# esteinig/sketchy

Measured on AMD Instinct MI355X. Metric: reads/sec streamed (s=10000,k=16,40k-genome ref), higher is better.
Workload: dtype u64

## Files before the change

sketchy_amd/csrc/skx_capi.hip:

```cpp
#include <dlfcn.h>
#include <hip/hip_runtime.h>
#include <rccl/rccl.h>

#include <unistd.h>

#include <algorithm>
#include <atomic>
#include <chrono>
#include <cmath>
#include <condition_variable>
#include <cstdarg>
#include <cstdio>
#include <cstdlib>
#include <cstring>
#include <mutex>
#include <string>
#include <thread>
#include <unordered_map>
#include <vector>

#include "sketchy_hip.h"
#include "skx_common.hpp"
#include "skx_genome_groups.hpp"
#include "skx_kernels.hpp"
// ... 985 lines not shown
    u32 *d_hist = nullptr, *d_nprow = nullptr;
    u64* d_pcw = nullptr;
    u32 npat_pad = 0;
    skx::PatRows pat_rows() const { return skx::PatRows{d_hist, npat_pad, d_gain_l, d_nprow}; }
    skx::RareIndex rare_index() const {
        skx::RareIndex ri = ref->rare_index();
        if (!use_pat) { ri.prec = nullptr; ri.n_pat = 0; }
        if (!static_dense) { ri.qs = nullptr; ri.n_sd = 0; }
        return ri;
    }
    u32 *d_cbad = nullptr, *d_nqc = nullptr;
    u32 *d_spc_g0 = nullptr, *d_spc_grp = nullptr;
    u32 n_pad_c = 0, n_grp_c = 0, cand_seq = 0;
    struct PassSet {
        u64 *tab = nullptr;
        u32 *cand = nullptr;
        u64 *tabc = nullptr;
        u32 *ncand = nullptr;
        u32 *mode = nullptr, *any_full = nullptr, *nqc_total = nullptr;
        u32 *ext = nullptr;
        skx::SlotExtents smap_ext;
        u32 mqc_whole = 0xFFu;
        u64 *mc = nullptr;
        u64 *mqc = nullptr;
        u64 *rowany_c = nullptr;
        u32 *grp_any_c = nullptr;
        u32 *smap = nullptr;
        u32 *pair_qc = nullptr;
        u32 *nd = nullptr;
        u32 *h_pub = nullptr;
    } ps[2];
    struct PassChains {
        bool pending = false, ranked = false, has_cand = false, update_table = false, forced_full = false, legacy = false;
        SubPass subs[kGroupMax];
        int n_sub = 0, b = 0, slot = 0;
        u32 P = 0, nq_rows = 0, seq = 0;
        u64 nq_est = 0;
    } pcq[2];
    int pc_head = 0, pc_n = 0;
    bool hint_all_overflow = false;
    u32 hint_seq = 0;
    u32 passes_since_fresh = 0;
    bool fresh_table = true;
    u32 legacy_run = 0;
    u64 batches_compact = 0, batches_full = 0;
    bool have_split_hint = false;
    double nd_frac = 1.0;
    u32 qcap_max = 0;
    bool qcap_auto = false;
    u64 qrows_grown = 0;
    u32 coalesce = 1;
    u32 rpass = 0;
    u64 reads_total = 0;
    uint8_t* d_bases = nullptr;
    u64* d_offsets = nullptr;
    u64* d_sk = nullptr;
    u32 *d_len = nullptr, *d_cnt = nullptr, *d_poff = nullptr;
    bool side_ready[kSides] = {};
    u64* sd_sk[kSides] = {};
    u64 pool_cap[kSides] = {};
    u32 pool_fixed = 0;
    u64* sd_rows[kSides] = {};
    u32 cur_stride = 0;
    u32 cur_pool_cap = 0, cur_pool_fixed = 0;
    u32 *sd_len[kSides] = {}, *sd_cnt[kSides] = {}, *sd_poff[kSides] = {}, *sd_big[kSides] = {};
    u32 *sd_chk[kSides] = {}, *sd_retry[kSides] = {};
// ... 9 lines not shown
    bool m_filled[2] = {false, false};
    u32* d_mdirty_s = nullptr;
    u32 sd64 = 0;
    u32 qhash_cap() const { return qcap - sd64; }
    struct RankLane {
        hipStream_t s = nullptr;
        u32 *d_inc = nullptr;
        u32 *d_csum_raw = nullptr;
        u32 *d_csum = nullptr;
        u32 *d_rel = nullptr;
        u32 *d_leader = nullptr;
        u64 *d_lead_val = nullptr;
        u64 *d_gmax = nullptr;
        u64 *d_lpart_sum = nullptr;
        u32 *d_lpart_idx = nullptr;
        u32 *d_live_ctr = nullptr;
        u64 *d_lead_seg = nullptr;
        unsigned char *d_has = nullptr;
        unsigned char *d_live = nullptr;
        u64 *d_cand_sum = nullptr;
        u32 *d_cand_idx = nullptr;
        u64 *d_cum_sink = nullptr;
        u32 *d_chg_flag = nullptr, *d_chg_pos = nullptr, *d_chg_bsum = nullptr, *d_chg_codes = nullptr;
        u32 *d_call_flag = nullptr, *d_call_pos = nullptr, *d_call_bsum = nullptr, *d_call_key = nullptr;
        u32 *d_call_sp = nullptr, *d_call_idx = nullptr, *d_call_codes = nullptr;
        u64* d_call_sum = nullptr;
        u32 call_key_w = 0;
        hipEvent_t ev_cum = nullptr;
        hipEvent_t ev_done = nullptr;
        bool ready = false;
    };
    static const int kRankLanes = kRankLanesMax;
    RankLane lane[kRankLanes];
    int n_lanes = 1;
    bool own_lane_stream = false;
    u32 n_cand_units = 0;
    u64 rank_seq = 0;
    RankLane* cum_writer = nullptr;
    u64* d_tab[kRankLanes + 1] = {};
    int tab_cur = 0;
    u64* d_cum = nullptr;
    u32* d_topk_idx = nullptr;
    u64* d_topk_sum = nullptr;
    u32* bound_cons = nullptr;
    u32* d_cons = nullptr;
    ChangeOut bound_chg;
    ChangeOut d_ev;
    CallOut bound_call;
    CallOut d_call;
    u64* d_tab_tmp = nullptr;
    u32* d_rank_idx = nullptr;
    u64* d_rank_sum = nullptr;
    u32 rank_cap = 0;
    StreamStats stats;
    u32* h_poff = nullptr;
    u64* h_offsets = nullptr;
    u64* d_ht[2] = {nullptr, nullptr};
    u32 ht_slots = 0;
    u32 *d_slot_off = nullptr, *d_bcount = nullptr, *d_bbase = nullptr, *d_btot = nullptr, *d_dict_ctr[2] = {nullptr, nullptr};
    u32* d_chk = nullptr;
    u32* h_chk = nullptr;
    u32* h_chk_base = nullptr;
    u32 pub_seq = 0;
    bool chk_dirty[kSides] = {};
    u64* d_rowany[2] = {nullptr, nullptr};
    u32* d_mqext = nullptr;
// ... 18 lines not shown
        u32 n_reads = 0;
        u64 n_bases = 0, ticket = 0;
        u32* out_idx = nullptr;
        u64* out_sum = nullptr;
        u32* out_cons = nullptr;
        u32* d_cons = nullptr;
        ChangeOut out_chg;
        ChangeOut d_ev;
        u32* h_ev_n = nullptr;
        CallOut out_call;
        CallOut d_call;
        u32* h_cev_n = nullptr;
        u32* d_rows_idx = nullptr;
        u64* d_rows_sum = nullptr;
        uint8_t* d_bases = nullptr;
        u64 *d_offsets = nullptr, *h_offsets = nullptr;
        hipEvent_t ev_copy = nullptr, ev_done = nullptr;
    } slot[kSlotsMax];
    u32 n_slots = 3;
    hipStream_t hs_copy = nullptr;
    u64 next_ticket = 0;
    u32* h_nq = nullptr;
    u32 hint_pairs[2] = {0, 0};
    double nq_per_pair = 1.0;
    bool have_hint = false;
    int profiling = 0;
    std::vector<TimedSpan> spans;
    std::vector<hipEvent_t> ev_pool;
    double ms[SKX_N_STAGES] = {0, 0, 0, 0, 0};
    u64 launches[SKX_N_STAGES] = {0, 0, 0, 0, 0};
};

static void free_side(skx_stream* st, int i);
static void free_lane(skx_stream* st, int i);
static void free_call(CallOut& d) {
    void* ptrs[] = {d.sp, d.idx, d.sum, d.codes, d.n_events, d.ev_read, d.ev_sp, d.ev_idx, d.ev_sum, d.ev_codes};
    for (void* q : ptrs) (void)hipFree(q);
    d = CallOut{};
}
static void stream_free(skx_stream* st) {
    if (!st) return;
    (void)hipSetDevice(st->device);
    if (st->hs0) (void)hipStreamSynchronize(st->hs0);
    if (st->hs1) (void)hipStreamSynchronize(st->hs1);
    if (st->hs) (void)hipStreamSynchronize(st->hs);
    if (st->hs2) (void)hipStreamSynchronize(st->hs2);
    for (int i = 1; i < skx_stream::kRankLanes; ++i)
        if (st->lane[i].s) (void)hipStreamSynchronize(st->lane[i].s);
    for (int i = 0; i < kSides; ++i) (void)hipFree(st->sd_rows[i]);
    void* ptrs[] = {st->d_bases, st->d_offsets, st->d_pair_h[0], st->d_pair_h[1],
                    st->d_q[0], st->d_q[1], st->d_pair_r[0], st->d_pair_r[1], st->d_pair_q[0], st->d_pair_q[1],
                    st->d_poff_pass[0], st->d_poff_pass[1], st->d_poff_pass[2], st->d_pair_r[2], st->d_nq[0], st->d_nq[1], st->d_win[0], st->d_win[1], st->d_m, st->d_mint, st->d_mq[0], st->d_mq[1],
                    st->d_topk_idx, st->d_topk_sum, st->d_cons, st->d_ev.n_events, st->d_ev.ev_read, st->d_ev.ev_idx, st->d_ev.ev_sum, st->d_ev.ev_codes, st->d_tab_tmp, st->d_rank_idx, st->d_rank_sum, st->d_bsum, st->d_grp_any[0],
                    st->d_grp_any[1], st->d_hbuf, st->d_wb[0], st->d_wb[1], st->d_rowany[0], st->d_rowany[1], st->d_mqext,
                    st->d_qd, st->d_qrow, st->d_sslot, st->d_qinfo, st->d_qloc, st->d_cls_bsum, st->d_nd_hs,
                    st->d_rowcnt, st->d_gain, st->d_gain_s, st->d_candslot, st->d_candmask, st->d_lrow, st->d_gop, st->d_gop_pairs, st->d_nlrow, st->d_gain_l, st->d_cbase, st->d_cwl, st->d_ncwl, st->d_cw, st->d_cbad, st->d_nqc, st->d_spc_g0, st->d_spc_grp, st->d_inb, st->d_hit, st->d_hist, st->d_nprow, st->d_pcw, st->d_ms[0], st->d_ms[1], st->d_mdirty_s};
    for (auto& q : st->ps) {
        for (void* x : {(void*)q.tab, (void*)q.cand, (void*)q.tabc, (void*)q.ncand, (void*)q.mode, (void*)q.any_full, (void*)q.nqc_total, (void*)q.mc, (void*)q.mqc,
                        (void*)q.rowany_c, (void*)q.grp_any_c, (void*)q.smap, (void*)q.pair_qc, (void*)q.nd}) (void)hipFree(x);
        if (q.h_pub) (void)hipHostFree(q.h_pub);
    }
    for (auto& t : st->d_tab) (void)hipFree(t);
    for (int i = 0; i < skx_stream::kRankLanes; ++i) free_lane(st, i);
    for (int i = 1; i < skx_stream::kRankLanes; ++i)
        if (st->own_lane_stream && st->lane[i].s) (void)hipStreamDestroy(st->lane[i].s);
    for (void* p : ptrs) (void)hipFree(p);
    stats_free(st->stats);
    if (st->h_poff) (void)hipHostFree(st->h_poff);
    if (st->h_offsets) (void)hipHostFree(st->h_offsets);
    if (st->h_nq) (void)hipHostFree(st->h_nq);
    if (st->h_nd) (void)hipHostFree(st->h_nd);
    if (st->h_nq_sink) (void)hipHostFree(st->h_nq_sink);
    if (st->h_lcount) (void)hipHostFree(st->h_lcount);
    if (st->h_chk_base) (void)hipHostFree(st->h_chk_base);
    for (int i = 0; i < kSides; ++i) {
        free_side(st, i);
        if (st->ev_main[i]) (void)hipEventDestroy(st->ev_main[i]);
    }
    if (!st->shared_queues && st->hs1 && st->hs1 != st->hs0) (void)hipStreamDestroy(st->hs1);
    (void)hipFree(st->d_ht[0]); (void)hipFree(st->d_ht[1]); (void)hipFree(st->d_dict_ctr[0]); (void)hipFree(st->d_dict_ctr[1]);
    (void)hipFree(st->d_slot_off); (void)hipFree(st->d_bcount); (void)hipFree(st->d_bbase);
    (void)hipFree(st->d_btot);
    free_call(st->d_call);
    for (auto& sl : st->slot) {
        free_call(sl.d_call);
        if (sl.h_cev_n) (void)hipHostFree(sl.h_cev_n);
        (void)hipFree(sl.d_bases); (void)hipFree(sl.d_offsets); (void)hipFree(sl.d_rows_idx); (void)hipFree(sl.d_rows_sum); (void)hipFree(sl.d_cons);
        (void)hipFree(sl.d_ev.n_events); (void)hipFree(sl.d_ev.ev_read); (void)hipFree(sl.d_ev.ev_idx); (void)hipFree(sl.d_ev.ev_sum); (void)hipFree(sl.d_ev.ev_codes);
        if (sl.h_ev_n) (void)hipHostFree(sl.h_ev_n);
        if (sl.h_offsets) (void)hipHostFree(sl.h_offsets);
        if (sl.ev_copy) (void)hipEventDestroy(sl.ev_copy);
        if (sl.ev_done) (void)hipEventDestroy(sl.ev_done);
    }
    if (st->hs_copy) (void)hipStreamDestroy(st->hs_copy);
    for (auto& sp : st->spans) { (void)hipEventDestroy(sp.a); (void)hipEventDestroy(sp.b); }
    for (auto ev : st->ev_pool) (void)hipEventDestroy(ev);
// ... 60 lines not shown
        if ((e = hipMalloc(&lr.list, (size_t)lr.long_cap * 4)) != hipSuccess) return e;
        if ((e = hipMalloc(&lr.seg0, (size_t)lr.long_cap * 4)) != hipSuccess) return e;
        if ((e = hipMalloc(&lr.seg_tab, (size_t)lr.segs_cap * 4)) != hipSuccess) return e;
        if ((e = hipMalloc(&lr.seg_cnt, (size_t)lr.segs_cap * 4)) != hipSuccess) return e;
        if ((e = hipMalloc(&lr.seg_h, (size_t)lr.segs_cap * skx::long_read_seg_slots() * 8)) != hipSuccess) return e;
    }
    return hipMemset(st->sd_big[i], 0, 4);
}
static hipError_t use_side(skx_stream* st, int i) {
    if (!st->side_ready[i]) {
        hipError_t e = alloc_side(st, i);
        if (e == hipSuccess) e = hipDeviceSynchronize();
        if (e != hipSuccess) return e;
    }
    st->side = i;
    st->d_sk = st->sd_sk[i]; st->cur_stride = 0; st->cur_pool_cap = (u32)st->pool_cap[i]; st->cur_pool_fixed = st->pool_fixed;
    st->d_len = st->sd_len[i]; st->d_cnt = st->sd_cnt[i]; st->d_poff = st->sd_poff[i];
    st->d_big = st->sd_big[i]; st->d_retry = st->sd_retry[i]; st->d_chk = st->sd_chk[i];
    st->lr = st->sd_lr[i];
    st->h_chk = st->h_chk_base + 16 * i;
    return hipSuccess;
}

static hipError_t use_rows(skx_stream* st) {
    const int i = st->side;
    if (!st->sd_rows[i]) {
        hipError_t e = hipMalloc(&st->sd_rows[i], (size_t)st->max_reads * st->sk_stride * 8);
        if (e != hipSuccess) return e;
    }
    st->d_sk = st->sd_rows[i]; st->cur_stride = st->sk_stride; st->cur_pool_cap = 0; st->cur_pool_fixed = 0;
    return hipSuccess;
}

static hipError_t alloc_lane_parts(skx_stream* st, int i) {
    skx_stream::RankLane& L = st->lane[i];
    const skx_ref* ref = st->ref;
    const u32 n_sp = ref->n_species, top_k = st->top_k, n_pad = std::max<u32>(ref->n_pad, n_sp * skx::kCandCap);
    const u32 n_seg_max = (st->rpass + skx::kSegLen - 1) / skx::kSegLen, n_chunk_max = (n_seg_max + 15) / 16;
    const u32 k1 = std::max<u32>(top_k, 1);
    hipError_t e;
#define LCHK(expr) do { if ((e = (expr)) != hipSuccess) return e; } while (0)
    LCHK(hipMalloc(&L.d_inc, (size_t)n_seg_max * n_pad * 4));
    LCHK(hipMalloc(&L.d_rel, (size_t)n_seg_max * n_pad * 4));
    LCHK(hipMalloc(&L.d_live, (size_t)n_seg_max * (n_pad / 64)));
    LCHK(hipMalloc(&L.d_has, (size_t)n_seg_max * (n_pad / (skx::kRankWords * 64))));
    LCHK(hipMalloc(&L.d_lead_seg, (size_t)n_seg_max * n_sp * 8 + 64));
    LCHK(hipMalloc(&L.d_live_ctr, 8));
    LCHK(hipMemset(L.d_live_ctr, 0, 8));
    LCHK(hipMalloc(&L.d_csum, (size_t)n_chunk_max * n_pad * 4));
    LCHK(hipMalloc(&L.d_csum_raw, (size_t)n_chunk_max * n_pad * 4));
    LCHK(hipMalloc(&L.d_leader, (size_t)n_chunk_max * n_sp * k1 * 4 + 64));
    LCHK(hipMalloc(&L.d_lead_val, (size_t)n_chunk_max * n_sp * 8 + 64));
    LCHK(hipMalloc(&L.d_lpart_sum, (size_t)n_chunk_max * n_sp * skx::rank_leader_parts() * k1 * 8 + 64));
    LCHK(hipMalloc(&L.d_lpart_idx, (size_t)n_chunk_max * n_sp * skx::rank_leader_parts() * k1 * 4 + 64));
    LCHK(hipMalloc(&L.d_gmax, (size_t)(n_chunk_max + 1) * (n_pad / 256) * 8 + 64));
    if (top_k) {
        LCHK(hipMalloc(&L.d_cand_sum, (size_t)st->rpass * st->n_cand_units * top_k * 8));
        LCHK(hipMalloc(&L.d_cand_idx, (size_t)st->rpass * st->n_cand_units * top_k * 4));
    }
    LCHK(hipMalloc(&L.d_cum_sink, (size_t)n_pad * 8));
    LCHK(hipEventCreateWithFlags(&L.ev_cum, hipEventDisableTiming));
    LCHK(hipEventCreateWithFlags(&L.ev_done, hipEventDisableTiming));
#undef LCHK
    return hipSuccess;
}
static void free_lane(skx_stream* st, int i) {
    skx_stream::RankLane& L = st->lane[i];
    void* ptrs[] = {L.d_inc, L.d_rel, L.d_live, L.d_has, L.d_lead_seg, L.d_live_ctr, L.d_csum, L.d_csum_raw, L.d_leader, L.d_lead_val,
                    L.d_lpart_sum, L.d_lpart_idx, L.d_gmax, L.d_cand_sum, L.d_cand_idx, L.d_cum_sink,
                    L.d_chg_flag, L.d_chg_pos, L.d_chg_bsum, L.d_chg_codes,
                    L.d_call_flag, L.d_call_pos, L.d_call_bsum, L.d_call_key, L.d_call_sp, L.d_call_idx, L.d_call_codes, L.d_call_sum};
    for (void* q : ptrs) (void)hipFree(q);
    if (L.ev_cum) (void)hipEventDestroy(L.ev_cum);
    if (L.ev_done) (void)hipEventDestroy(L.ev_done);
    const hipStream_t keep = L.s;
    L = skx_stream::RankLane{};
    L.s = keep;
}
static hipError_t alloc_lane(skx_stream* st, int i) {
    const hipError_t e = alloc_lane_parts(st, i);
    if (e != hipSuccess) { free_lane(st, i); (void)hipGetLastError(); }
    else st->lane[i].ready = true;
    return e;
}

static int stream_create_internal(skx_stream** out, const skx_ref* ref, u32 top_k, u32 max_reads, u64 max_bases,
                                  u32 sk_stride, u32 pair_hint, bool dense_queries = false, bool enqueueing = false) {
    SKXCHK(use_device(ref->device));
    skx_stream* st = new skx_stream;
    st->ref = ref; st->device = ref->device; st->top_k = top_k; st->max_reads = max_reads; st->max_bases = max_bases;
    st->sk_stride = sk_stride;
    const u32 n_pad = ref->n_pad, n_gw = n_pad / 64;
    static const u64 pass_pairs_env = skx::knob("SKX_PASS_PAIRS") ? (u64)atoll(skx::knob("SKX_PASS_PAIRS")) : 0;
    u64 pc = std::min<u64>((u64)max_reads * std::min<u32>(sk_stride, pair_hint), 1u << 22);
    if (pass_pairs_env) pc = pass_pairs_env;
    pc = std::max<u64>(pc, sk_stride);
    pc = (pc + 63) / 64 * 64;
    st->pcap = (u32)pc;
    const u32 rows_policy = g_stream_query_rows.load();
    u64 qc = rows_policy ? rows_policy : 65536;
    if (!rows_policy && ref->static_dense) qc += (ref->n_sd + 63u) & ~63u;
    if (dense_queries) {
        size_t mem_free = 0, mem_total = 0;
        (void)hipMemGetInfo(&mem_free, &mem_total);
        qc = std::max<u64>(qc, std::min<u64>(pc, (u64)(mem_free / 6) / (3ull * n_pad / 8)));
    }
    qc = std::max<u64>(std::min<u64>(qc, pc), std::min<u64>(pc, sk_stride));
    qc = (qc + 63) / 64 * 64;
    st->qcap = (u32)qc;
    st->qcap_auto = rows_policy == 0 && !dense_queries;
    st->qcap_max = st->qcap;
    if (st->qcap_auto) {
        size_t mem_free = 0, mem_total = 0;
        (void)hipMemGetInfo(&mem_free, &mem_total);
        const u64 per_row = (u64)n_pad / 8 + 2ull * ((n_gw + skx::kRankWords - 1) / skx::kRankWords * skx::kRankWords) * 8 + 3ull * skx::kPassBatchesMax * 4 + 8;
// ... 122 lines not shown
        SCHK(hipMemset(st->d_mq[i], 0, bytes));
    }
    {
        const u32 any[4] = {skx::mq_any_stride(), 0xFFFFFFFFu, skx::mq_any_stride(), 0xFFFFFFFFu};
        SCHK(hipMalloc(&st->d_mqext, sizeof(any)));
        SCHK(hipMemcpy(st->d_mqext, any, sizeof(any), hipMemcpyHostToDevice));
    }
    st->n_cand_units = n_cand_units;
    {
        static const int lanes_env = skx::knob("SKX_RANK_LANES") ? atoi(skx::knob("SKX_RANK_LANES")) : 0;
        const int want = lanes_env ? lanes_env : (int)g_rank_lanes;
        st->n_lanes = (enqueueing && top_k && st->depth >= 3) ? std::max(1, std::min(want, (int)skx_stream::kRankLanes)) : 1;
        st->lane[0].s = st->hs2;
        for (int i = 1; i < st->n_lanes; ++i) {
            if (st->shared_queues) {
                hipError_t lane_err = hipSuccess;
                {
                    std::lock_guard<std::mutex> lk(g_queues_mu);
                    SharedQueues& q = g_queues[st->device & 63];
                    static const int rank_hi_l = skx::knob("SKX_PRIO_RANK") ? atoi(skx::knob("SKX_PRIO_RANK")) : 0;
                    const int prio_rank_l = rank_hi_l == 1 ? prio_hi : rank_hi_l == 2 ? (prio_lo + prio_hi) / 2 : prio_lo;
                    if (!q.lane_s[i - 1]) {
                        lane_err = hipStreamCreateWithPriority(&q.lane_s[i - 1], hipStreamNonBlocking, prio_rank_l);
                        if (lane_err != hipSuccess) q.lane_s[i - 1] = nullptr;
                    }
                    st->lane[i].s = q.lane_s[i - 1];
                }
                SCHK(lane_err);
            } else {
                SCHK(hipStreamCreateWithPriority(&st->lane[i].s, hipStreamNonBlocking, prio_lo));
                st->own_lane_stream = true;
            }
        }
        SCHK(alloc_lane(st, 0));
        for (int i = 1; i < st->n_lanes; ++i)
            if (alloc_lane(st, i) != hipSuccess) { st->n_lanes = i; break; }
    }
    for (int i = 0; i <= st->n_lanes; ++i) {
        SCHK(hipMalloc(&st->d_tab[i], (size_t)n_pad * 8));
        SCHK(hipMemset(st->d_tab[i], 0, (size_t)n_pad * 8));
    }
    st->tab_cur = 0;
    st->d_cum = st->d_tab[0];
    if (top_k) {
        SCHK(hipMalloc(&st->d_topk_idx, (size_t)max_reads * n_sp * top_k * 4));
        SCHK(hipMalloc(&st->d_topk_sum, (size_t)max_reads * n_sp * top_k * 8));
    }
    SCHK(hipMalloc(&st->d_tab_tmp, (size_t)ref->n_genomes * 8));
    st->rank_cap = n_sp * std::max<u32>(SKX_MAX_TOP, top_k);
    SCHK(hipMalloc(&st->d_rank_idx, (size_t)st->rank_cap * 4));
    SCHK(hipMalloc(&st->d_rank_sum, (size_t)st->rank_cap * 8));
    SCHK(hipMalloc(&st->d_bsum, ((size_t)max_reads / 1024 + 2) * 4));
    for (int i = 0; i < 2; ++i) SCHK(hipMalloc(&st->d_grp_any[i], (size_t)(n_pad / (skx::kRankWords * 64) + 1) * 4));
    for (int i = 0; i < 2; ++i) {
        SCHK(hipMalloc(&st->d_rowany[i], (size_t)(n_pad / (skx::kRankWords * 64)) * (st->qcap / 64 + 2) * 8));
        SCHK(hipMemset(st->d_rowany[i], 0, (size_t)(n_pad / (skx::kRankWords * 64)) * (st->qcap / 64 + 2) * 8));
    }
    if (skx::scan_lean_wants_slabs() && skx::scan_lean_applies(ref->n_bands, false, false)) {
        SCHK(hipMalloc(&st->d_hbuf, (size_t)n_bt * skx::scan_lean_words() * skx::kTileGenomes * 8));
        for (int i = 0; i < 2; ++i) SCHK(hipMalloc(&st->d_wb[i], ((size_t)st->qcap / 64 + 1) * ref->n_tiles * 16));
    }
    SCHK(hipHostMalloc((void**)&st->h_poff, ((size_t)max_reads + 2) * 4, hipHostMallocDefault));
    SCHK(hipHostMalloc((void**)&st->h_offsets, ((size_t)max_reads + 1) * 8, hipHostMallocDefault));
    st->ht_slots = 1024;
    while (st->ht_slots < 2ull * st->pcap) st->ht_slots <<= 1;
    for (int i = 0; i < 2; ++i) {
        SCHK(hipMalloc(&st->d_ht[i], (size_t)st->ht_slots * 8));
        SCHK(hipMemset(st->d_ht[i], 0xFF, (size_t)st->ht_slots * 8));
        SCHK(hipMalloc(&st->d_dict_ctr[i], 64));
// ... 561 lines not shown
        }
        seq = ++st->cand_seq;
        skx::launch_cand_publish(hs, st->d_cbad, force_full, ps.ncand, st->d_nqc, d_nd, (u32)n_sub, n_sp, rows_c, ps.mode, ps.any_full,
                                 ps.nqc_total, ps.h_pub, seq, fill_mqc ? ps.ext : nullptr);
        st->front_open = false;
        if (ranked && P > 0 && !all_forced)
            skx::launch_cand_gather_m(hs, d_m, m_int, n_pad, d_nd, sdm ? ref->n_sd : q_bound, ps.cand, st->n_pad_c, st->d_cbad, (u32)n_sub, ps.mc, rows_c / 64);
        only_if = ps.any_full;
        HIPCHK(hipGetLastError());
    }
    if (P > 0) {
        static const int direct_env = skx::knob("SKX_RARE_DIRECT") ? atoi(skx::knob("SKX_RARE_DIRECT")) : 1;
        const bool direct_rare = split_dict && ref->rare_direct && (direct_env != 0 || sdm);
        if (split_dict && !direct_rare) {
            Span sp(st, 1, hs);
            skx::launch_sparse_fill(hs, st->d_sslot, d_nd, st->rare_index(), d_m, n_pad, d_mdirty, q_bound, only_if);
        }
        if (!direct_rare) HIPCHK(hipMemsetAsync(st->d_mqext + 2 * b, 0, 8, hs));
        {
            Span sp(st, 3, hs);
            skx::launch_transpose_bits(hs, d_m, split ? st->d_mint : nullptr, n_pad, n_words, d_mq, direct_rare ? d_nd + 2 : d_nd + 3, d_grp_any,
                                       nullptr, st->d_wb[b], d_win, ref->n_tiles, d_mdirty, direct_rare ? nd_est : nq_est, st->d_rowany[b], only_if,
                                       sdm && st->reuse_m);
            if (direct_rare)
                skx::launch_rare_to_mq(hs, st->d_sslot, d_nd, st->rare_index(), d_mq, nq_rows, n_pad, st->d_rowany[b], d_grp_any, q_bound, only_if,
                                       st->d_mqext + 2 * b);
            if (only_if && !(sdm && st->reuse_m)) skx::launch_m_clear(hs, d_m, split ? st->d_mint : nullptr, n_pad, d_nd, only_if);
        }
        if (sdm) st->m_ready[b] = false;
    }
    HIPCHK(hipGetLastError());
    HIPCHK(hipEventRecord(st->ev_front[b], hs));
    st->front_pending[b] = true;
    (void)lean_used;

    SKXCHK(queue_chains(st, false));
    skx_stream::PassChains& pc = st->pcq[(st->pc_head + st->pc_n) & 1];
    st->pc_n += 1;
    pc.pending = true; pc.ranked = ranked; pc.has_cand = update_table;
    pc.n_sub = n_sub; pc.b = b; pc.slot = slot; pc.P = P; pc.nq_rows = nq_rows; pc.seq = seq; pc.nq_est = nq_est;
    for (int i = 0; i < n_sub; ++i) pc.subs[i] = subs[i];
    pc.update_table = update_table;
    pc.forced_full = all_forced || legacy;
    pc.legacy = legacy;
    if (legacy) { pc.has_cand = false; all_forced = true; }
    SKX_MARK("pass: scan + transpose queued", 0);
    if (all_forced) SKXCHK(queue_chains(st, true));
    return SKX_OK;
}

static int queue_one(skx_stream* st, skx_stream::PassChains& pc, bool block, bool* done);
static void update_cand_hint(skx_stream* st) {
    {
        volatile u32* hl = st->h_lcount;
        const u32 seq = hl[1], count = hl[0];
        if (seq != st->lcount_seen && (int)(seq - st->lcount_floor) > 0 && hl[1] == seq) {
            st->hint_all_overflow = count > skx::kCandCap && st->top_k != 0;
            st->lcount_seen = seq;
        }
    }
    for (auto& q : st->ps) {
        volatile u32* hp = q.h_pub;
        const u32 seq = hp[2 * skx::kPassBatchesMax + 1], n_b = hp[2 * skx::kPassBatchesMax + 2];
        if (seq == 0 || (int)(seq - st->hint_seq) <= 0 || n_b == 0 || n_b > skx::kPassBatchesMax) continue;
        bool all_over = true;
        for (u32 i = 0; i < n_b; ++i) all_over = all_over && hp[skx::kPassBatchesMax + i] >= skx::kCandCap;
        if (hp[2 * skx::kPassBatchesMax + 1] != seq) continue;
        st->hint_all_overflow = all_over && st->top_k != 0;
        st->hint_seq = seq;
    }
}
static int queue_chains_until(skx_stream* st, int leave) {
    while (st->pc_n > leave) {
        bool done = false;
        SKXCHK(queue_one(st, st->pcq[st->pc_head], true, &done));
        st->pc_head ^= 1; st->pc_n -= 1;
    }
    return SKX_OK;
}
static int queue_chains(skx_stream* st, bool block) {
    if (block) return queue_chains_until(st, 0);
    while (st->pc_n > 0) {
        bool done = false;
        SKXCHK(queue_one(st, st->pcq[st->pc_head], false, &done));
        if (!done) break;
        st->pc_head ^= 1; st->pc_n -= 1;
    }
    return SKX_OK;
}
static int queue_one(skx_stream* st, skx_stream::PassChains& pc, bool block, bool* done) {
    *done = false;
    if (!pc.pending) { *done = true; return SKX_OK; }
    const skx_ref* ref = st->ref;
    const int b = pc.b, slot = pc.slot, n_sub = pc.n_sub;
    skx_stream::PassSet& ps = st->ps[b];
    u32 mode[kGroupMax] = {};
    if (pc.has_cand && !pc.forced_full) {
        volatile u32* hp = ps.h_pub;
        if (hp[2 * skx::kPassBatchesMax + 1] != pc.seq) {
            if (!block) return SKX_OK;
            SKX_T0();
            for (u64 spins = 0; hp[2 * skx::kPassBatchesMax + 1] != pc.seq; ++spins)
                if ((spins & 0xFFFFu) == 0xFFFFu) {
                    const hipError_t e = hipStreamQuery(st->hs);
                    if (e != hipSuccess && e != hipErrorNotReady) return fail(SKX_ERR_HIP, "the scan stream failed: %s", hipGetErrorString(e));
                    if (e == hipSuccess && hp[2 * skx::kPassBatchesMax + 1] != pc.seq) {
                        (void)hipGetLastError();
                        if (hp[2 * skx::kPassBatchesMax + 1] != pc.seq) return fail(SKX_ERR_HIP, "internal: the pass's candidates were never published");
                    }
                    (void)hipGetLastError();
                }
            SKX_ACC(wait);
        }
        for (int i = 0; i < n_sub; ++i) mode[i] = hp[i];
    }
    update_cand_hint(st);
    pc.pending = false;
    *done = true;
    hipStream_t hs2 = st->hs2;
    const skx::Species spc = ref->species();
    const u32 n_pad = ref->n_pad, n_sp = ref->n_species;
    const u32 nq_rows = pc.nq_rows, P = pc.P;
    const bool update_table = pc.update_table;
    u32 *d_pair_r = st->d_pair_r[slot], *d_pair_q = st->d_pair_q[b];
    u64* d_mq = st->d_mq[b];
    u32* d_grp_any = st->d_grp_any[b];
    u32* const d_nq_rows = ps.nd + 3;
    bool lane_used[skx_stream::kRankLanes] = {};
    for (int si = 0; si < n_sub; ++si) {
    SKX_MARK("rank: begin sub", si);
    const SubPass& sb = pc.subs[si];
    const int li = (update_table && n_sub > 1) ? (int)(st->rank_seq % (u64)st->n_lanes) : 0;
    skx_stream::RankLane& L = st->lane[li];
    hipStream_t ls = L.s;
    if (!lane_used[li]) { HIPCHK(hipStreamWaitEvent(ls, st->ev_front[b], 0)); lane_used[li] = true; }
    const u32 n_reads = sb.rb - sb.ra, sub_base = sb.p_base;
    u32* const d_topk_idx = sb.d_topk_idx;
    u64* const d_topk_sum = sb.d_topk_sum;
    const u32 out_r0 = sb.ra;
    const u32 n_seg = (n_reads + skx::kSegLen - 1) / skx::kSegLen;
    const bool ranked = st->top_k && d_topk_idx && d_topk_sum;
    const bool compact = update_table && ranked && mode[si] == 1u;
    const u32 c_pad = compact ? st->n_pad_c : n_pad, c_gw = c_pad / 64, c_rows = compact ? skx::kCandRows : nq_rows;
    const skx::Species c_spc = compact ? skx::Species{st->d_spc_g0, ps.ncand + (size_t)si * n_sp, st->d_spc_grp, n_sp} : spc;
    const u64* c_mq = compact ? ps.mqc + (size_t)si * st->n_grp_c * skx::kCandRows * skx::kRankWords : d_mq;
    u32* c_grp_any = compact ? ps.grp_any_c + (size_t)si * st->n_grp_c : d_grp_any;
    const u64* c_rowany = compact ? ps.rowany_c + (size_t)si * st->n_grp_c * (skx::kCandRows / 64) : (P > 0 ? st->d_rowany[b] : nullptr);
    const u32* c_nq = compact ? ps.nqc_total + si : d_nq_rows;
    const bool legacy = pc.legacy && update_table;
    if (legacy && st->cum_writer && st->cum_writer != &L) HIPCHK(hipStreamWaitEvent(ls, st->cum_writer->ev_cum, 0));
    int tab_next = st->tab_cur;
    if (legacy) {
        do { tab_next = (tab_next + 1) % (st->n_lanes + 1); } while (st->d_tab[tab_next] == st->d_cum);
    }
    const u64* const cum_in = legacy ? st->d_cum : update_table ? (compact ? ps.tabc + (size_t)si * st->n_pad_c : ps.tab + (size_t)si * n_pad) : st->d_cum;
    const u32 *sub_pair_q = (compact ? ps.pair_qc : d_pair_q) + sb.p_off, *sub_pair_r = d_pair_r + sb.p_off, *sub_poff = sb.d_poff;
    if (update_table && ranked) { if (compact) st->batches_compact += 1; else st->batches_full += 1; }
    if (compact) {
        Span sp(st, 3, ls);
        if (P > 0)
            skx::launch_transpose_bits(ls, ps.mc + (size_t)si * (skx::kCandRows / 64) * st->n_pad_c, nullptr, st->n_pad_c, skx::kCandRows / 64,
                                       const_cast<u64*>(c_mq), ps.nd, c_grp_any, nullptr, nullptr, nullptr, 0, nullptr, pc.nq_est,
                                       const_cast<u64*>(c_rowany));
        skx::launch_cand_pair_rows(ls, d_pair_q + sb.p_off, sb.P, ps.nd, ps.smap + (size_t)si * ((size_t)st->qcap + 128), skx::kCandRows,
                                   ps.pair_qc + sb.p_off);
        HIPCHK(hipGetLastError());
    }
    const u32 prune_k = (ranked && st->top_k <= skx::rank_topk_fast_max()) ? st->top_k : 0u;
    static const int two_level_env = skx::knob("SKX_TWO_LEVEL") ? atoi(skx::knob("SKX_TWO_LEVEL")) : -1;
    const volatile u32* h_live = st->h_nq + 2;
    const u32 live_now = h_live[0], tested_now = h_live[1];
    static const u32 live_pct_env = skx::knob("SKX_LIVE_PCT") ? (u32)atoi(skx::knob("SKX_LIVE_PCT")) : 33u;
    const bool mostly_dead = tested_now != 0 && (u64)live_now * 100 < (u64)tested_now * live_pct_env;
    const bool two_level = !compact && prune_k != 0 && (two_level_env >= 0 ? two_level_env != 0 : mostly_dead);
    u32 *d_inc = L.d_inc, *d_csum_raw = L.d_csum_raw;
// ... 134 lines not shown
                    c_sum = L.d_call_sum;
                }
                if (co.ev_codes && !c_codes) {
                    if (!L.d_call_codes) HIPCHK(hipMalloc(&L.d_call_codes, mr * nf * 4));
                    c_codes = L.d_call_codes;
                }
            }
            const bool key_codes = co.ev_codes != nullptr;
            skx::launch_species_call(ls, d_topk_idx, d_topk_sum, d_codes, sb.ra, sb.rb, n_sp, st->top_k, nf, c_sp, c_idx, c_sum, c_codes, c_key,
                                     key_codes);
            if (co.cap) {
                skx::launch_change_flags(ls, c_key, 1u + (key_codes ? nf : st->top_k), sb.ra, sb.rb, L.d_call_flag);
                if (sb.rb == co.n_batch) {
                    skx::launch_change_events(ls, L.d_call_flag, L.d_call_pos, L.d_call_bsum, co.n_batch, co.cap, co.n_events, co.ev_read,
                                              co.ev_idx ? c_idx : nullptr, co.ev_sum ? c_sum : nullptr, st->top_k, co.ev_idx, co.ev_sum,
                                              co.ev_codes ? c_codes : nullptr, nf, co.ev_codes);
                    if (co.ev_sp) skx::launch_call_species_gather(ls, L.d_call_flag, L.d_call_pos, co.n_batch, co.cap, c_sp, co.ev_sp);
                }
            }
        }
    }
    if (sb.d_shared)
        skx::launch_shared_debug(ls, d_pair_q + sb.p_off, sub_poff, sub_base, 0, n_reads, d_mq, nq_rows, ref->n_genomes, ref->d_real2pad, sb.d_shared, 0);
    if (sb.d_counts) {
        HIPCHK(hipMemsetAsync(sb.d_counts, 0, (size_t)n_reads * n_pad * 4, ls));
        if (P > 0)
            skx::launch_seg_sum(ls, d_pair_q + sb.p_off, sub_poff, sub_base, 0, n_reads, 1, d_mq, n_pad, nq_rows, sb.d_counts, d_grp_any, nullptr,
                                st->d_rowany[b], d_nq_rows, spc);
    }
    HIPCHK(hipGetLastError());
    SKX_MARK("rank: end sub", si);
    }
    if (!lane_used[0]) HIPCHK(hipStreamWaitEvent(hs2, st->ev_front[b], 0));
    for (int li = 1; li < st->n_lanes; ++li)
        if (lane_used[li]) {
            HIPCHK(hipEventRecord(st->lane[li].ev_done, st->lane[li].s));
            HIPCHK(hipStreamWaitEvent(hs2, st->lane[li].ev_done, 0));
        }
    HIPCHK(hipEventRecord(st->ev_back[b], hs2));
    st->back_pending[b] = true;
    HIPCHK(hipEventRecord(st->ev_pslot[slot], hs2));
    st->pslot_pending[slot] = true;
    int rc = SKX_OK;
    for (int si = 0; si < n_sub; ++si) {
        const int r2 = staged_rows(st, pc.subs[si].slot);
        if (rc == SKX_OK && r2 != SKX_OK) rc = r2;
    }
    return rc;
}

static int run_pass(skx_stream* st, u32 ra, u32 rb, u32 p_base, u32 P, u32* d_topk_idx, u64* d_topk_sum,
                    u32* d_shared , bool update_table, bool inserted = false, u32 q_rows = 0xFFFFFFFFu,
                    void* slot = nullptr, u32* d_counts = nullptr , u32* d_cons = nullptr,
                    const ChangeOut* chg = nullptr, const CallOut* call = nullptr) {
    SubPass sb;
    sb.slot = slot; sb.d_cons = d_cons;
    if (chg) sb.chg = *chg;
    if (call) sb.call = *call;
    sb.ra = ra; sb.rb = rb; sb.p_off = 0; sb.P = P; sb.p_base = p_base; sb.d_topk_idx = d_topk_idx; sb.d_topk_sum = d_topk_sum;
    sb.d_shared = d_shared; sb.d_counts = d_counts; sb.side = st->side;
    sb.d_poff = st->d_poff_pass[st->pslot];
    return run_pass_multi(st, &sb, 1, update_table, inserted, q_rows);
}

template <class F>
static int for_each_pass(skx_stream* st, u32 n_reads, u32 max_pass_reads, F fn) {
    const u32 cap = std::max<u32>(1u, std::min<u32>(st->rpass, max_pass_reads));
    const u32 pair_cap = std::min(st->pcap, st->qhash_cap());
    u32 ra = 0;
    while (ra < n_reads) {
// ... 394 lines not shown
        subs[i].d_poff = st->d_poff_pass[g[0].spec_slot] + (size_t)i * ((size_t)st->rpass + 2);
        subs[i].slot = g[i].slot; subs[i].d_cons = g[i].d_cons; subs[i].chg = g[i].chg; subs[i].call = g[i].call;
        p_off += P[i];
    }
    st->last_pairs = pairs; st->last_passes = 1; st->shared_passes += 1;
    {
        SKX_T0();
        SKXCHK(run_pass_multi(st, subs, n, true, true, q_rows));
        SKX_ACC(back);
    }
    st->reads_total += reads;
    *n_done = n;
    return SKX_OK;
}

static int staged_rows(skx_stream* st, void* slot);
static void staged_drop(void* slot);
static int pending_back(skx_stream* st, PendingBatch* younger) {
    PendingBatch g[kGroupMax];
    const int n = st->n_pend;
    for (int i = 0; i < n; ++i) g[i] = st->pend[i];
    st->n_pend = 0;
    if (n == 0) return SKX_OK;
    int done = 0;
    st->tail_pass = younger == nullptr;
    int rc = batch_back_group(st, g, n, younger, &done);
    st->tail_pass = false;
    const std::string msg = rc != SKX_OK ? g_err : std::string();
    for (int i = done; i < n; ++i) staged_drop(g[i].slot);
    if (!msg.empty()) g_err = msg;
    return rc;
}
static int flush_pending(skx_stream* st) {
    const int rc = pending_back(st, nullptr);
    const std::string msg = rc != SKX_OK ? g_err : std::string();
    const int rc2 = queue_chains(st, true);
    if (rc != SKX_OK) { g_err = msg; return rc; }
    return rc2;
}
static int process_batch(skx_stream* st, const uint8_t* d_bases, const u64* d_offsets, u32 n_reads, u64 n_bases, u32* d_topk_idx,
                         u64* d_topk_sum, u32* h_shared, u64* h_sketches, u32* h_sketch_len, u32* d_cons = nullptr,
                         const ChangeOut* chg = nullptr, const CallOut* call = nullptr) {
    if (n_reads == 0) return SKX_OK;
    SKXCHK(flush_pending(st));
    PendingBatch pb;
    pb.d_bases = d_bases; pb.d_offsets = d_offsets; pb.n_reads = n_reads; pb.n_bases = n_bases;
    pb.d_topk_idx = d_topk_idx; pb.d_topk_sum = d_topk_sum;
    pb.h_shared = h_shared; pb.h_sketches = h_sketches; pb.h_sketch_len = h_sketch_len; pb.d_cons = d_cons;
    if (chg) { pb.chg = *chg; pb.chg.n_batch = n_reads; }
    if (call) { pb.call = *call; pb.call.n_batch = n_reads; }
    SKXCHK(batch_front(st, pb));
    st->tail_pass = true;
    const int rc = batch_back(st, pb, nullptr);
    st->tail_pass = false;
    return rc;
}
static int enqueue_batch(skx_stream* st, const uint8_t* d_bases, const u64* d_offsets, u32 n_reads, u64 n_bases, u32* d_topk_idx,
                         u64* d_topk_sum, void* slot, u32* d_cons, const ChangeOut* chg = nullptr, const CallOut* call = nullptr) {
    PendingBatch nw;
    nw.d_cons = d_cons;
    if (chg) { nw.chg = *chg; nw.chg.n_batch = n_reads; }
    if (call) { nw.call = *call; nw.call.n_batch = n_reads; }
    nw.d_bases = d_bases; nw.d_offsets = d_offsets; nw.n_reads = n_reads; nw.n_bases = n_bases;
    nw.d_topk_idx = d_topk_idx; nw.d_topk_sum = d_topk_sum; nw.slot = slot;
    nw.pairable = st->coalesce >= 2;
    nw.max_group = slot ? std::min<u32>(st->coalesce, kStagedGroupMax) : st->coalesce;
// ... 1706 lines not shown
SKX_API int skx_comm_n_ranks(const skx_comm* comm, int* n_ranks) {
    if (!comm || !n_ranks) return fail(SKX_ERR_INVALID, "NULL argument");
    *n_ranks = comm->n_ranks;
    if (g_rccl.CommCount) {
        int n = 0;
        ncclResult_t r = g_rccl.CommCount(comm->comm, &n);
        if (r != ncclSuccess) return fail(SKX_ERR_COMM, "ncclCommCount: %s", g_rccl.GetErrorString ? g_rccl.GetErrorString(r) : "?");
        *n_ranks = n;
    }
    return SKX_OK;
}
SKX_API int skx_stream_allreduce(skx_stream* st, skx_comm* comm) {
    if (!st || !comm) return fail(SKX_ERR_INVALID, "NULL argument");
    if (comm->device != st->device) return fail(SKX_ERR_INVALID, "communicator and stream are on different devices");
    SKXCHK(use_device(st->device));
    SKXCHK(flush_pending(st));
    CommWatchdog wd(g_comm_timeout_ms, "ncclAllReduce of the running table", comm->rank, comm->n_ranks, comm->device);
    ncclResult_t r = g_rccl.AllReduce(st->d_cum, st->d_cum, st->ref->n_pad, ncclUint64, ncclSum, comm->comm, st->hs2);
    if (r != ncclSuccess) return fail(SKX_ERR_COMM, "ncclAllReduce: %s", g_rccl.GetErrorString ? g_rccl.GetErrorString(r) : "?");
    HIPCHK(hipStreamSynchronize(st->hs2));
    return SKX_OK;
}
SKX_API void skx_comm_destroy(skx_comm* comm) {
    if (!comm) return;
    if (g_rccl.CommDestroy) (void)g_rccl.CommDestroy(comm->comm);
    delete comm;
}

#ifdef SKX_EXPERIMENTS
namespace skx { void rank_debug_counters(unsigned long long* out, bool reset); }
namespace skx { void gain_dense_launches(unsigned long long* out, bool reset); }
SKX_API void skx_debug_rank_counters(unsigned long long* out, int reset) { skx::rank_debug_counters(out, reset != 0); }
SKX_API void skx_debug_gain_launches(unsigned long long* out, int reset) { skx::gain_dense_launches(out, reset != 0); }
SKX_API int skx_debug_row_topk(int device, const uint32_t* counts, uint32_t n_rows, uint32_t n, uint32_t top_k, uint32_t bound,
                               uint32_t* top_idx, uint32_t* top_val) {
    if (!counts || !top_idx || !top_val || n_rows < 1 || n < 1) return fail(SKX_ERR_INVALID, "skx_debug_row_topk: bad argument");
    if (top_k < 1 || top_k > SKX_MAX_TOP || top_k > n) return fail(SKX_ERR_INVALID, "skx_debug_row_topk: top_k=%u outside 1..min(n, SKX_MAX_TOP)", top_k);
    SKXCHK(use_device(device));
    const u32 n_pad = (n + kGroupGenomes - 1) / kGroupGenomes * kGroupGenomes;
    DevMem m_cnt, m_sp, m_idx, m_val;
    HIPCHK(m_cnt.need((size_t)n_rows * n_pad * 4));
    HIPCHK(m_sp.need(2 * 4));
    HIPCHK(m_idx.need((size_t)n_rows * top_k * 4));
    HIPCHK(m_val.need((size_t)n_rows * top_k * 4));
    const u32 sp_host[2] = {0u, n};
    HIPCHK(hipMemset(m_cnt.p, 0xFF, (size_t)n_rows * n_pad * 4));
    HIPCHK(hipMemcpy2D(m_cnt.p, (size_t)n_pad * 4, counts, (size_t)n * 4, (size_t)n * 4, n_rows, hipMemcpyHostToDevice));
    HIPCHK(hipMemcpy(m_sp.p, sp_host, sizeof sp_host, hipMemcpyHostToDevice));
    const skx::Species sp{m_sp.as<u32>(), m_sp.as<u32>() + 1, nullptr, 1};
    skx::launch_row_topk(nullptr, m_cnt.as<u32>(), n_rows, n_pad, sp, top_k, bound, m_idx.as<u32>(), m_val.as<u32>());
    HIPCHK(hipGetLastError());
    HIPCHK(hipMemcpy(top_idx, m_idx.p, (size_t)n_rows * top_k * 4, hipMemcpyDeviceToHost));
    HIPCHK(hipMemcpy(top_val, m_val.p, (size_t)n_rows * top_k * 4, hipMemcpyDeviceToHost));
    return SKX_OK;
}
SKX_API int skx_debug_ref_rows(const skx_ref* ref, uint32_t species, uint32_t first, uint32_t count, uint64_t* rows, uint32_t* len) {
    if (!ref || !rows || !len || species >= ref->n_species) return fail(SKX_ERR_INVALID, "skx_debug_ref_rows: bad argument");
    if (count < 1 || first > ref->sp_n[species] || count > ref->sp_n[species] - first) return fail(SKX_ERR_INVALID, "skx_debug_ref_rows: bad range");
    SKXCHK(use_device(ref->device));
    DevMem m_rows, m_len;
    HIPCHK(m_rows.need((size_t)count * ref->s * 8));
    HIPCHK(m_len.need((size_t)count * 4));
    HIPCHK(hipMemset(m_rows.p, 0xA5, (size_t)count * ref->s * 8));
    skx::launch_ref_rows(nullptr, ref->d_mat, ref->s, ref->sp_g0[species] + first, count, ref->d_exc_g, ref->d_exc_h, ref->n_exc, m_rows.as<u64>(), ref->s,
                         m_len.as<u32>());
    HIPCHK(hipGetLastError());
// ... 6 lines not shown
```

Measured before the change: 165.8 million.

## Spread tail-pass compact rank sub-passes across extra lanes on idle front streams

Adds up to three compact-only rank lanes bound to the front-side streams (hs0, hs1, hs). During tail passes (flush, or when no further fronts are queued), compact sub-passes without change or call outputs are spread round-robin across the regular rank lanes and these tail lanes. The goal is to parallelise the serialized rank chain at the end of streaming, when the front streams have nothing else to run. In exchange it allocates extra lane buffers and adds cross-stream event waits, and it only engages when the queues are not shared with another stream.

```diff
diff --git a/sketchy_amd/csrc/skx_capi.hip b/sketchy_amd/csrc/skx_capi.hip
--- a/sketchy_amd/csrc/skx_capi.hip
+++ b/sketchy_amd/csrc/skx_capi.hip
@@ -1041,6 +1041,8 @@
     } ps[2];
     struct PassChains {
         bool pending = false, ranked = false, has_cand = false, update_table = false, forced_full = false, legacy = false;
+        bool tail = false;
+        u32 front_no = 0;
         SubPass subs[kGroupMax];
         int n_sub = 0, b = 0, slot = 0;
         u32 P = 0, nq_rows = 0, seq = 0;
@@ -1116,6 +1118,10 @@
     };
     static const int kRankLanes = kRankLanesMax;
     RankLane lane[kRankLanes];
+    static const int kTailLanes = 3;
+    RankLane tail[kTailLanes];
+    int n_tail = 0;
+    u32 fronts_queued = 0;
     int n_lanes = 1;
     bool own_lane_stream = false;
     u32 n_cand_units = 0;
@@ -1200,7 +1206,7 @@
 };
 
 static void free_side(skx_stream* st, int i);
-static void free_lane(skx_stream* st, int i);
+static void free_lane(skx_stream::RankLane& L);
 static void free_call(CallOut& d) {
     void* ptrs[] = {d.sp, d.idx, d.sum, d.codes, d.n_events, d.ev_read, d.ev_sp, d.ev_idx, d.ev_sum, d.ev_codes};
     for (void* q : ptrs) (void)hipFree(q);
@@ -1229,7 +1235,8 @@
         if (q.h_pub) (void)hipHostFree(q.h_pub);
     }
     for (auto& t : st->d_tab) (void)hipFree(t);
-    for (int i = 0; i < skx_stream::kRankLanes; ++i) free_lane(st, i);
+    for (int i = 0; i < skx_stream::kRankLanes; ++i) free_lane(st->lane[i]);
+    for (auto& t : st->tail) free_lane(t);
     for (int i = 1; i < skx_stream::kRankLanes; ++i)
         if (st->own_lane_stream && st->lane[i].s) (void)hipStreamDestroy(st->lane[i].s);
     for (void* p : ptrs) (void)hipFree(p);
@@ -1356,11 +1363,14 @@
     return hipSuccess;
 }
 
-static hipError_t alloc_lane_parts(skx_stream* st, int i) {
-    skx_stream::RankLane& L = st->lane[i];
+static hipError_t alloc_lane_parts(skx_stream* st, skx_stream::RankLane& L, bool compact_only) {
     const skx_ref* ref = st->ref;
-    const u32 n_sp = ref->n_species, top_k = st->top_k, n_pad = std::max<u32>(ref->n_pad, n_sp * skx::kCandCap);
-    const u32 n_seg_max = (st->rpass + skx::kSegLen - 1) / skx::kSegLen, n_chunk_max = (n_seg_max + 15) / 16;
+    const u32 n_sp = ref->n_species, top_k = st->top_k;
+    const u32 n_pad = compact_only ? n_sp * skx::kCandCap : std::max<u32>(ref->n_pad, n_sp * skx::kCandCap);
+    const u32 n_units = !compact_only ? st->n_cand_units
+                        : (top_k >= 1 && top_k <= skx::rank_topk_fast_max()) ? (n_pad / 64 + skx::kRankWords - 1) / skx::kRankWords : n_pad / 64;
+    const u32 n_seg_max = compact_only ? ((st->rpass + skx::kSegLen - 1) / skx::kSegLen + 15u) / 16u * 16u : (st->rpass + skx::kSegLen - 1) / skx::kSegLen;
+    const u32 n_chunk_max = (n_seg_max + 15) / 16;
     const u32 k1 = std::max<u32>(top_k, 1);
     hipError_t e;
 #define LCHK(expr) do { if ((e = (expr)) != hipSuccess) return e; } while (0)
@@ -1379,8 +1389,8 @@
     LCHK(hipMalloc(&L.d_lpart_idx, (size_t)n_chunk_max * n_sp * skx::rank_leader_parts() * k1 * 4 + 64));
     LCHK(hipMalloc(&L.d_gmax, (size_t)(n_chunk_max + 1) * (n_pad / 256) * 8 + 64));
     if (top_k) {
-        LCHK(hipMalloc(&L.d_cand_sum, (size_t)st->rpass * st->n_cand_units * top_k * 8));
-        LCHK(hipMalloc(&L.d_cand_idx, (size_t)st->rpass * st->n_cand_units * top_k * 4));
+        LCHK(hipMalloc(&L.d_cand_sum, (size_t)st->rpass * n_units * top_k * 8));
+        LCHK(hipMalloc(&L.d_cand_idx, (size_t)st->rpass * n_units * top_k * 4));
     }
     LCHK(hipMalloc(&L.d_cum_sink, (size_t)n_pad * 8));
     LCHK(hipEventCreateWithFlags(&L.ev_cum, hipEventDisableTiming));
@@ -1388,8 +1398,7 @@
 #undef LCHK
     return hipSuccess;
 }
-static void free_lane(skx_stream* st, int i) {
-    skx_stream::RankLane& L = st->lane[i];
+static void free_lane(skx_stream::RankLane& L) {
     void* ptrs[] = {L.d_inc, L.d_rel, L.d_live, L.d_has, L.d_lead_seg, L.d_live_ctr, L.d_csum, L.d_csum_raw, L.d_leader, L.d_lead_val,
                     L.d_lpart_sum, L.d_lpart_idx, L.d_gmax, L.d_cand_sum, L.d_cand_idx, L.d_cum_sink,
                     L.d_chg_flag, L.d_chg_pos, L.d_chg_bsum, L.d_chg_codes,
@@ -1401,10 +1410,10 @@
     L = skx_stream::RankLane{};
     L.s = keep;
 }
-static hipError_t alloc_lane(skx_stream* st, int i) {
-    const hipError_t e = alloc_lane_parts(st, i);
-    if (e != hipSuccess) { free_lane(st, i); (void)hipGetLastError(); }
-    else st->lane[i].ready = true;
+static hipError_t alloc_lane(skx_stream* st, skx_stream::RankLane& L, bool compact_only = false) {
+    const hipError_t e = alloc_lane_parts(st, L, compact_only);
+    if (e != hipSuccess) { free_lane(L); (void)hipGetLastError(); }
+    else L.ready = true;
     return e;
 }
 
@@ -1593,9 +1602,19 @@
                 st->own_lane_stream = true;
             }
         }
-        SCHK(alloc_lane(st, 0));
+        SCHK(alloc_lane(st, st->lane[0]));
         for (int i = 1; i < st->n_lanes; ++i)
-            if (alloc_lane(st, i) != hipSuccess) { st->n_lanes = i; break; }
+            if (alloc_lane(st, st->lane[i]) != hipSuccess) { st->n_lanes = i; break; }
+        static const bool tail_env = !skx::knob("SKX_TAIL_LANES") || atoi(skx::knob("SKX_TAIL_LANES")) != 0;
+        st->n_tail = 0;
+        if (tail_env && st->n_lanes >= 2 && st->depth == 3 && st->hs0 != st->hs1 && st->hs0 != st->hs && st->hs1 != st->hs) {
+            const hipStream_t ts[skx_stream::kTailLanes] = {st->hs0, st->hs1, st->hs};
+            for (int i = 0; i < skx_stream::kTailLanes; ++i) {
+                if (alloc_lane(st, st->tail[i], true) != hipSuccess) break;
+                st->tail[i].s = ts[i];
+                st->n_tail = i + 1;
+            }
+        }
     }
     for (int i = 0; i <= st->n_lanes; ++i) {
         SCHK(hipMalloc(&st->d_tab[i], (size_t)n_pad * 8));
@@ -2223,6 +2242,7 @@
     HIPCHK(hipGetLastError());
     HIPCHK(hipEventRecord(st->ev_front[b], hs));
     st->front_pending[b] = true;
+    st->fronts_queued += 1;
     (void)lean_used;
 
     SKXCHK(queue_chains(st, false));
@@ -2232,6 +2252,7 @@
     pc.n_sub = n_sub; pc.b = b; pc.slot = slot; pc.P = P; pc.nq_rows = nq_rows; pc.seq = seq; pc.nq_est = nq_est;
     for (int i = 0; i < n_sub; ++i) pc.subs[i] = subs[i];
     pc.update_table = update_table;
+    pc.tail = st->tail_pass; pc.front_no = st->fronts_queued;
     pc.forced_full = all_forced || legacy;
     pc.legacy = legacy;
     if (legacy) { pc.has_cand = false; all_forced = true; }
@@ -2261,6 +2282,17 @@
         st->hint_seq = seq;
     }
 }
+static bool sole_queue_user(const skx_stream* st) {
+    if (!st->shared_queues) return true;
+    std::lock_guard<std::mutex> lk(g_queues_mu);
+    return g_queues[st->device & 63].refs == 1;
+}
+#ifdef SKX_EXPERIMENTS
+static std::atomic<unsigned long long> g_chain_lanes[kRankLanesMax + skx_stream::kTailLanes];
+static inline void chain_queued(int li) { g_chain_lanes[li].fetch_add(1, std::memory_order_relaxed); }
+#else
+static inline void chain_queued(int) {}
+#endif
 static int queue_chains_until(skx_stream* st, int leave) {
     while (st->pc_n > leave) {
         bool done = false;
@@ -2317,14 +2349,17 @@
     u64* d_mq = st->d_mq[b];
     u32* d_grp_any = st->d_grp_any[b];
     u32* const d_nq_rows = ps.nd + 3;
-    bool lane_used[skx_stream::kRankLanes] = {};
+    bool lane_used[skx_stream::kRankLanes + skx_stream::kTailLanes] = {};
+    int spread_ring[skx_stream::kRankLanes + skx_stream::kTailLanes], n_ring = 0;
+    if (pc.tail && update_table && !pc.legacy && n_sub > 1 && st->n_tail > 0 && sole_queue_user(st)) {
+        for (int i = 0; i < st->n_lanes; ++i) spread_ring[n_ring++] = i;
+        for (int i = 0; i < st->n_tail; ++i)
+            if (i < 2 || pc.front_no == st->fronts_queued) spread_ring[n_ring++] = skx_stream::kRankLanes + i;
+    }
+    int n_spread = 0;
     for (int si = 0; si < n_sub; ++si) {
     SKX_MARK("rank: begin sub", si);
     const SubPass& sb = pc.subs[si];
-    const int li = (update_table && n_sub > 1) ? (int)(st->rank_seq % (u64)st->n_lanes) : 0;
-    skx_stream::RankLane& L = st->lane[li];
-    hipStream_t ls = L.s;
-    if (!lane_used[li]) { HIPCHK(hipStreamWaitEvent(ls, st->ev_front[b], 0)); lane_used[li] = true; }
     const u32 n_reads = sb.rb - sb.ra, sub_base = sb.p_base;
     u32* const d_topk_idx = sb.d_topk_idx;
     u64* const d_topk_sum = sb.d_topk_sum;
@@ -2332,6 +2367,12 @@
     const u32 n_seg = (n_reads + skx::kSegLen - 1) / skx::kSegLen;
     const bool ranked = st->top_k && d_topk_idx && d_topk_sum;
     const bool compact = update_table && ranked && mode[si] == 1u;
+    const bool spread = n_ring > 0 && compact && !sb.chg.cap && !sb.call.any();
+    const int li = spread ? spread_ring[n_spread++ % n_ring] : (update_table && n_sub > 1) ? (int)(st->rank_seq % (u64)st->n_lanes) : 0;
+    skx_stream::RankLane& L = li < skx_stream::kRankLanes ? st->lane[li] : st->tail[li - skx_stream::kRankLanes];
+    hipStream_t ls = L.s;
+    if (!lane_used[li]) { HIPCHK(hipStreamWaitEvent(ls, st->ev_front[b], 0)); lane_used[li] = true; }
+    chain_queued(li);
     const u32 c_pad = compact ? st->n_pad_c : n_pad, c_gw = c_pad / 64, c_rows = compact ? skx::kCandRows : nq_rows;
     const skx::Species c_spc = compact ? skx::Species{st->d_spc_g0, ps.ncand + (size_t)si * n_sp, st->d_spc_grp, n_sp} : spc;
     const u64* c_mq = compact ? ps.mqc + (size_t)si * st->n_grp_c * skx::kCandRows * skx::kRankWords : d_mq;
@@ -2532,10 +2573,11 @@
     SKX_MARK("rank: end sub", si);
     }
     if (!lane_used[0]) HIPCHK(hipStreamWaitEvent(hs2, st->ev_front[b], 0));
-    for (int li = 1; li < st->n_lanes; ++li)
+    for (int li = 1; li < skx_stream::kRankLanes + skx_stream::kTailLanes; ++li)
         if (lane_used[li]) {
-            HIPCHK(hipEventRecord(st->lane[li].ev_done, st->lane[li].s));
-            HIPCHK(hipStreamWaitEvent(hs2, st->lane[li].ev_done, 0));
+            skx_stream::RankLane& J = li < skx_stream::kRankLanes ? st->lane[li] : st->tail[li - skx_stream::kRankLanes];
+            HIPCHK(hipEventRecord(J.ev_done, J.s));
+            HIPCHK(hipStreamWaitEvent(hs2, J.ev_done, 0));
         }
     HIPCHK(hipEventRecord(st->ev_back[b], hs2));
     st->back_pending[b] = true;
@@ -2996,6 +3038,7 @@
     return rc;
 }
 static int flush_pending(skx_stream* st) {
+    for (auto& q : st->pcq) if (q.pending) q.tail = true;
     const int rc = pending_back(st, nullptr);
     const std::string msg = rc != SKX_OK ? g_err : std::string();
     const int rc2 = queue_chains(st, true);
@@ -4768,6 +4811,12 @@
 namespace skx { void gain_dense_launches(unsigned long long* out, bool reset); }
 SKX_API void skx_debug_rank_counters(unsigned long long* out, int reset) { skx::rank_debug_counters(out, reset != 0); }
 SKX_API void skx_debug_gain_launches(unsigned long long* out, int reset) { skx::gain_dense_launches(out, reset != 0); }
+SKX_API void skx_debug_chain_lanes(unsigned long long* out, int reset) {
+    for (int i = 0; i < kRankLanesMax + skx_stream::kTailLanes; ++i) {
+        out[i] = g_chain_lanes[i].load(std::memory_order_relaxed);
+        if (reset) g_chain_lanes[i].store(0, std::memory_order_relaxed);
+    }
+}
 SKX_API int skx_debug_row_topk(int device, const uint32_t* counts, uint32_t n_rows, uint32_t n, uint32_t top_k, uint32_t bound,
                                uint32_t* top_idx, uint32_t* top_val) {
     if (!counts || !top_idx || !top_val || n_rows < 1 || n < 1) return fail(SKX_ERR_INVALID, "skx_debug_row_topk: bad argument");
```

New measurement: 164.5 million. About the same (-0.8%).
